# yeyupiaoling/VoiceprintRecognition-PaddlePaddle

Measured on AMD Instinct MI355X. Metric: utterances/sec (3 s, 16 kHz) ECAPA-TDNN fwd+AAM, higher is better.
Workload: dtype bf16; 1 GPU; BASELINE configs[1]: ECAPA-TDNN (C=512, MFA 1536, ASP, embd 192) + Kaldi Fbank 80, 3 s @ 16 kHz (T=298), 2796-class cosine head + AAMLoss, eval-mode forward, batch 256 per GPU, inputs resident in HBM, random-init weights; batch_per_gpu=256, global_batch=256, parallelism=dp1 (no collective), streams_per_gpu=2, hip_graph=True, graph_prereplays=40

## Files before the change

voiceprintrecognition-paddlepaddle_amd/csrc/head_tiled.hip:

```cpp
#include "head_common.h"

#include <math.h>

namespace {

constexpr int HT_CT = 64;
constexpr int HT_RB = 64;
constexpr int HT_RF = 32;
constexpr int HT_DMAX = 256;
constexpr int HT_SW = HT_CT + 2;
typedef __attribute__((ext_vector_type(4))) float v4f;

struct HeadTileArgs {
    const float* emb; const float* W; const long long* labels;
    float* part;
    float* tgt;
    float* cinv;
    const float* rinv;
    int B, D, C, tiles, SE;
    VpMargin mg; float scale; int easy;
    const float* mt;
};

__device__ __forceinline__ float row16_sum(float x) {
    x += __int_as_float(__builtin_amdgcn_update_dpp(0, __float_as_int(x), 0x128, 0xf, 0xf, false));
    x += __int_as_float(__builtin_amdgcn_update_dpp(0, __float_as_int(x), 0x124, 0xf, 0xf, false));
    x += __int_as_float(__builtin_amdgcn_update_dpp(0, __float_as_int(x), 0x122, 0xf, 0xf, false));
    x += __int_as_float(__builtin_amdgcn_update_dpp(0, __float_as_int(x), 0x121, 0xf, 0xf, false));
    return x;
}
__device__ __forceinline__ float row16_max(float x) {
    x = fmaxf(x, __int_as_float(__builtin_amdgcn_update_dpp(0, __float_as_int(x), 0x128, 0xf, 0xf, false)));
    x = fmaxf(x, __int_as_float(__builtin_amdgcn_update_dpp(0, __float_as_int(x), 0x124, 0xf, 0xf, false)));
    x = fmaxf(x, __int_as_float(__builtin_amdgcn_update_dpp(0, __float_as_int(x), 0x122, 0xf, 0xf, false)));
    x = fmaxf(x, __int_as_float(__builtin_amdgcn_update_dpp(0, __float_as_int(x), 0x121, 0xf, 0xf, false)));
    return x;
}


typedef __attribute__((ext_vector_type(4))) unsigned int ht_u32x4;
constexpr unsigned HT_OOB = 0xfffffff0u;

template <int NR>
__device__ __forceinline__ void ht_load_w(const float* W, int D, int C, int c0, int tid, float* Ws) {
    const int cq = (tid & 15) * 4, k0 = tid >> 4;
    if ((C & 3) == 0) {
        const __amdgpu_buffer_rsrc_t srd = __builtin_amdgcn_make_buffer_rsrc(const_cast<float*>(W), 0, (unsigned)((size_t)D * C * 4), 0x00020000);
        const bool cok = c0 + cq < C;
        ht_u32x4 v[NR];
#pragma unroll
        for (int i = 0; i < NR; ++i) {
            const int k = k0 + 16 * i;
            v[i] = __builtin_amdgcn_raw_buffer_load_b128(srd, (cok && k < D) ? (unsigned)(((size_t)k * C + c0 + cq) * 4) : HT_OOB, 0, 0);
        }
#pragma unroll
        for (int i = 0; i < NR; ++i) {
            const int k = k0 + 16 * i;
            if (k < D) {
                float* dst = Ws + k * HT_SW + cq;
                const ht_u32x4 t = v[i];
                dst[0] = __builtin_bit_cast(float, (unsigned)t[0]); dst[1] = __builtin_bit_cast(float, (unsigned)t[1]);
                dst[2] = __builtin_bit_cast(float, (unsigned)t[2]); dst[3] = __builtin_bit_cast(float, (unsigned)t[3]);
            }
        }
    } else {
        for (int k = k0; k < D; k += 16)
#pragma unroll
            for (int e = 0; e < 4; ++e) Ws[k * HT_SW + cq + e] = c0 + cq + e < C ? W[(size_t)k * C + c0 + cq + e] : 0.f;
    }
}

template <int NE, int ROWS = HT_RB>
__device__ __forceinline__ void ht_issue_e(const float* emb, int B, int D, int b0, int tid, ht_u32x4 (&v)[NE]) {
    const __amdgpu_buffer_rsrc_t srd = __builtin_amdgcn_make_buffer_rsrc(const_cast<float*>(emb), 0, (unsigned)((size_t)B * D * 4), 0x00020000);
    const int per_row = D >> 2, total = ROWS * per_row;
#pragma unroll
    for (int i = 0; i < NE; ++i) {
        const int idx = tid + 256 * i;
        const int r = idx / per_row, kq = (idx - r * per_row) * 4;
        v[i] = __builtin_amdgcn_raw_buffer_load_b128(srd, (idx < total && b0 + r < B) ? (unsigned)(((size_t)(b0 + r) * D + kq) * 4) : HT_OOB, 0, 0);
    }
}
template <int NE, int ROWS = HT_RB>
__device__ __forceinline__ void ht_commit_e(int D, int SE, int tid, float* Es, const ht_u32x4 (&v)[NE]) {
    const int per_row = D >> 2, total = ROWS * per_row;
#pragma unroll
    for (int i = 0; i < NE; ++i) {
        const int idx = tid + 256 * i;
        if (idx < total) {
            const int r = idx / per_row, kq = (idx - r * per_row) * 4;
            float* dst = Es + r * SE + kq;
            const ht_u32x4 t = v[i];
            dst[0] = __builtin_bit_cast(float, (unsigned)t[0]); dst[1] = __builtin_bit_cast(float, (unsigned)t[1]);
            dst[2] = __builtin_bit_cast(float, (unsigned)t[2]); dst[3] = __builtin_bit_cast(float, (unsigned)t[3]);
        }
    }
}
template <int NE, int ROWS = HT_RB>
__device__ __forceinline__ void ht_load_e(const float* emb, int B, int D, int SE, int b0, int tid, float* Es) {
    ht_u32x4 v[NE];
    ht_issue_e<NE, ROWS>(emb, B, D, b0, tid, v);
    ht_commit_e<NE, ROWS>(D, SE, tid, Es, v);
}

__global__ __launch_bounds__(256, 2) void head_tile_fwd_kernel(HeadTileArgs a) {
    extern __shared__ __attribute__((aligned(16))) char smem[];
    float* Ws = reinterpret_cast<float*>(smem);
    float* Es = Ws + a.D * HT_SW;
    float* cinv_s = Es + HT_RF * a.SE;
    float* rinv_s = cinv_s + HT_CT;
    float* red = rinv_s + HT_RF;
    int* lab_s = reinterpret_cast<int*>(red + 5 * 4 * HT_RF);
    vp_margin_override(a.mg, a.mt, false);
    const int tid = threadIdx.x, lane = tid & 63, wv = tid >> 6;
    const int li = lane & 15, g = lane >> 4;
    const int tile = blockIdx.x, c0 = tile * HT_CT;
    ht_load_w<HT_DMAX / 16>(a.W, a.D, a.C, c0, tid, Ws);
    __syncthreads();
    {
        const int c = tid & 63, q = tid >> 6;
        float s = 0.f;
        for (int k = q; k < a.D; k += 4) { const float v = Ws[k * HT_SW + c]; s += v * v; }
        red[q * 64 + c] = s;
        __syncthreads();
        if (tid < 64) {
            const float t = red[c] + red[64 + c] + red[128 + c] + red[192 + c];
            const float inv = 1.f / fmaxf(sqrtf(t), 1e-12f);
            cinv_s[c] = inv;
            if (a.cinv && c0 + c < a.C) a.cinv[c0 + c] = inv;
        }
    }
    const int cw = wv * 16;
    constexpr int NE = HT_RF * HT_DMAX / 4 / 256;
    ht_u32x4 ev[NE];
    if ((int)(blockIdx.y * HT_RF) < a.B) ht_issue_e<NE, HT_RF>(a.emb, a.B, a.D, blockIdx.y * HT_RF, tid, ev);
    for (int b0 = blockIdx.y * HT_RF; b0 < a.B; b0 += gridDim.y * HT_RF) {
        __syncthreads();
        if (tid < HT_RF) {
            lab_s[tid] = b0 + tid < a.B ? (int)a.labels[b0 + tid] : -1;
            rinv_s[tid] = b0 + tid < a.B ? a.rinv[b0 + tid] : 0.f;
        }
        ht_commit_e<NE, HT_RF>(a.D, a.SE, tid, Es, ev);
        __syncthreads();
        if (b0 + (int)gridDim.y * HT_RF < a.B) ht_issue_e<NE, HT_RF>(a.emb, a.B, a.D, b0 + gridDim.y * HT_RF, tid, ev);
        constexpr int MI = HT_RF / 16;
        v4f acc[MI];
#pragma unroll
        for (int mi = 0; mi < MI; ++mi) acc[mi] = v4f{0.f, 0.f, 0.f, 0.f};
        const float* wp = Ws + g * HT_SW + cw + li;
        const float* ep = Es + li * a.SE + g;
        const int se16 = 16 * a.SE;
        for (int k = 0; k < a.D; k += 16) {
            float bv[4], av[4][MI];
#pragma unroll
            for (int u = 0; u < 4; ++u) {
                const int kk = k + 4 * u < a.D ? k + 4 * u : 0;
                bv[u] = k + 4 * u < a.D ? wp[kk * HT_SW] : 0.f;
#pragma unroll
                for (int mi = 0; mi < MI; ++mi) av[u][mi] = ep[mi * se16 + kk];
            }
#pragma unroll
            for (int u = 0; u < 4; ++u)
#pragma unroll
                for (int mi = 0; mi < MI; ++mi) acc[mi] = __builtin_amdgcn_mfma_f32_16x16x4f32(av[u][mi], bv[u], acc[mi], 0, 0, 0);
        }
        const int c = c0 + cw + li;
        const bool cvalid = c < a.C;
        const float ci = cinv_s[cw + li];
#pragma unroll
        for (int mi = 0; mi < MI; ++mi) {
#pragma unroll
            for (int r = 0; r < 4; ++r) {
                const int row = mi * 16 + g * 4 + r;
                const int b = b0 + row;
                const int y = lab_s[row];
                const float cs = acc[mi][r] * rinv_s[row] * ci;
                float o = cs;
                if (c == y) o = vp_aam_margin(a.mg, a.easy, cs);
                o *= a.scale;
                if (c == y) a.tgt[b] = o;
                const float ov = cvalid ? o : -INFINITY;
                const float m = row16_max(ov);
                const float s = row16_sum(cvalid ? expf(o - m) : 0.f);
                const float so = row16_sum(cvalid ? o : 0.f);
                const float cv = cvalid ? cs : -INFINITY;
                const float bc = row16_max(cv);
                const float bi = -row16_max(cv == bc ? -(float)c : -INFINITY);
                if (li == 0) {
                    red[(0 * 4 + wv) * HT_RF + row] = m; red[(1 * 4 + wv) * HT_RF + row] = s; red[(2 * 4 + wv) * HT_RF + row] = so;
                    red[(3 * 4 + wv) * HT_RF + row] = bc; red[(4 * 4 + wv) * HT_RF + row] = bi;
                }
            }
        }
        __syncthreads();
        if (tid < HT_RF && b0 + tid < a.B) {
            const int row = tid;
            float M = fmaxf(fmaxf(red[0 * HT_RF + row], red[1 * HT_RF + row]), fmaxf(red[2 * HT_RF + row], red[3 * HT_RF + row]));
            float S = 0.f, O = 0.f;
#pragma unroll
            for (int w = 0; w < 4; ++w) {
                const float mw = red[(0 * 4 + w) * HT_RF + row];
                S += mw == -INFINITY ? 0.f : red[(1 * 4 + w) * HT_RF + row] * expf(mw - M);
                O += red[(2 * 4 + w) * HT_RF + row];
            }
            float BC = -INFINITY, BI = 0.f;
#pragma unroll
            for (int w = 0; w < 4; ++w) {
                const float v = red[(3 * 4 + w) * HT_RF + row];
                if (v > BC) { BC = v; BI = red[(4 * 4 + w) * HT_RF + row]; }
            }
            const size_t o = (size_t)(b0 + row) * a.tiles + tile;
            const size_t st = (size_t)a.B * a.tiles;
            a.part[o] = M;
            a.part[st + o] = S;
            a.part[2 * st + o] = O;
            a.part[3 * st + o] = BC;
            a.part[4 * st + o] = BI;
        }
    }
}

__global__ __launch_bounds__(256) void head_tile_merge_kernel(const float* part, const float* tgt, int B, int C, int tiles, float ls,
                                                              float* lse_out, float* row_loss, int* pred) {
    __shared__ float sm[5][4];
    const int b = blockIdx.x, tid = threadIdx.x, lane = tid & 63, wv = tid >> 6;
    const float* pm = part + (size_t)b * tiles;
    const float* ps = part + (size_t)B * tiles + (size_t)b * tiles;
    const float* po = part + 2 * (size_t)B * tiles + (size_t)b * tiles;
    const float* pc = part + 3 * (size_t)B * tiles + (size_t)b * tiles;
    const float* pi = part + 4 * (size_t)B * tiles + (size_t)b * tiles;
    float mx = -INFINITY, se = 0.f, so = 0.f, bc = -INFINITY, bi = 0.f;
    for (int t = tid; t < tiles; t += 256) {
        const float m = pm[t], s = ps[t];
        so += po[t];
        if (m > mx) { se = se * expf(mx - m) + s; mx = m; }
        else if (m != -INFINITY) se += s * expf(m - mx);
        const float v = pc[t];
        if (v > bc) { bc = v; bi = pi[t]; }
    }
    const float wbc = vp_wave_max(bc);
    const float wbi = -vp_wave_max(bc == wbc ? -bi : -INFINITY);
    if (lane == 0) { sm[3][wv] = wbc; sm[4][wv] = wbi; }
    float lse, O;
    vp_lse_merge(mx, se, so, sm, lse, O);
    if (tid == 0) {
        if (lse_out) lse_out[b] = lse;
        row_loss[b] = (1.f - ls) * (lse - tgt[b]) + ls * (lse - O / (float)C);
        if (pred) {
            float BC = -INFINITY, BI = 0.f;
            for (int w = 0; w < 4; ++w)
                if (sm[3][w] > BC || (sm[3][w] == BC && sm[4][w] < BI)) { BC = sm[3][w]; BI = sm[4][w]; }
            pred[b] = (int)BI;
        }
    }
}

constexpr int HT_SG = HT_CT + 2;

struct HeadBwdArgs {
    const float* emb; const float* W; const long long* labels; const float* lse;
    float* dW; float* dxn_part;
    int B, D, C, tiles, SE;
    VpMargin mg; float scale, ls, gscale; int easy;
    const float* mt;
};

template <int NKB>
__global__ __launch_bounds__(256) void head_tile_bwd_kernel(HeadBwdArgs a) {
    constexpr int D = 16 * NKB;
    constexpr int SE = D + 2;
    constexpr int KPW = NKB / 4;
    extern __shared__ __attribute__((aligned(16))) char smem[];
    float* Ws = reinterpret_cast<float*>(smem);
    float* Es = Ws + D * HT_SW;
    float* Gs = Es + HT_RB * SE;
    float* cinv_s = Gs + HT_RB * HT_SG;
    float* rinv_s = cinv_s + HT_CT;
    float* lse_s = rinv_s + HT_RB;
    float* red = lse_s + HT_RB;
    int* lab_s = reinterpret_cast<int*>(red + 4 * 64);
    vp_margin_override(a.mg, a.mt, false);
    const int tid = threadIdx.x, lane = tid & 63, wv = tid >> 6;
    const int li = lane & 15, g = lane >> 4;
    const int cw = wv * 16;
    const float kk = a.gscale / (float)a.B * a.scale;
    const float qoff = a.ls / (float)a.C;
    const int nrb = (a.B + HT_RB - 1) / HT_RB;
    v4f dxn[2][4][KPW];
#pragma unroll
    for (int rb = 0; rb < 2; ++rb)
#pragma unroll
        for (int mi = 0; mi < 4; ++mi)
#pragma unroll
            for (int kb = 0; kb < KPW; ++kb) dxn[rb][mi][kb] = v4f{0.f, 0.f, 0.f, 0.f};
    for (int tile = blockIdx.x; tile < a.tiles; tile += gridDim.x) {
        const int c0 = tile * HT_CT;
        __syncthreads();
        ht_load_w<NKB>(a.W, D, a.C, c0, tid, Ws);
        __syncthreads();
        {
            const int c = tid & 63, q = tid >> 6;
            float s = 0.f;
            for (int k = q; k < D; k += 4) { const float v = Ws[k * HT_SW + c]; s += v * v; }
            red[q * 64 + c] = s;
            __syncthreads();
            if (tid < 64) cinv_s[c] = 1.f / fmaxf(sqrtf(red[c] + red[64 + c] + red[128 + c] + red[192 + c]), 1e-12f);
        }
        v4f dwn[NKB];
#pragma unroll
        for (int kb = 0; kb < NKB; ++kb) dwn[kb] = v4f{0.f, 0.f, 0.f, 0.f};
#pragma unroll
        for (int rb = 0; rb < 2; ++rb) {
            if (rb < nrb) {
                const int b0 = rb * HT_RB;
                __syncthreads();
                if (tid < HT_RB) {
                    const bool ok = b0 + tid < a.B;
                    lab_s[tid] = ok ? (int)a.labels[b0 + tid] : -1;
                    lse_s[tid] = ok ? a.lse[b0 + tid] : 0.f;
                }
                ht_load_e<HT_RB * D / 4 / 256>(a.emb, a.B, D, SE, b0, tid, Es);
                __syncthreads();
                {
                    const int r = tid & 63, q = tid >> 6;
                    float s = 0.f;
                    for (int k = q; k < D; k += 4) { const float v = Es[r * SE + k]; s += v * v; }
                    red[q * 64 + r] = s;
                    __syncthreads();
                    if (tid < 64) rinv_s[r] = 1.f / fmaxf(sqrtf(red[r] + red[64 + r] + red[128 + r] + red[192 + r]), 1e-12f);
                    __syncthreads();
                }
                v4f acc[4];
#pragma unroll
                for (int mi = 0; mi < 4; ++mi) acc[mi] = v4f{0.f, 0.f, 0.f, 0.f};
                {
                    const float* wp = Ws + g * HT_SW + cw + li;
                    const float* ep = Es + li * SE + g;
                    for (int k = 0; k < D; k += 16) {
                        float bv[4], av[4][4];
#pragma unroll
                        for (int u = 0; u < 4; ++u) {
                            bv[u] = wp[(k + 4 * u) * HT_SW];
#pragma unroll
                            for (int mi = 0; mi < 4; ++mi) av[u][mi] = ep[mi * 16 * SE + k + 4 * u];
                        }
#pragma unroll
                        for (int u = 0; u < 4; ++u)
#pragma unroll
                            for (int mi = 0; mi < 4; ++mi) acc[mi] = __builtin_amdgcn_mfma_f32_16x16x4f32(av[u][mi], bv[u], acc[mi], 0, 0, 0);
                    }
                }
                {
                    const int c = c0 + cw + li;
                    const bool cvalid = c < a.C;
                    const float ci = cinv_s[cw + li];
#pragma unroll
                    for (int mi = 0; mi < 4; ++mi)
#pragma unroll
                        for (int r = 0; r < 4; ++r) {
                            const int row = mi * 16 + g * 4 + r;
                            const int y = lab_s[row];
                            const float cs = acc[mi][r] * rinv_s[row] * ci;
                            float o = cs, dm = 1.f;
                            if (c == y) o = vp_aam_margin(a.mg, a.easy, cs, dm);
                            o *= a.scale;
                            const float q = qoff + (c == y ? 1.f - a.ls : 0.f);
                            const float gv = (cvalid && y >= 0) ? kk * (expf(o - lse_s[row]) - q) * dm * ci : 0.f;
                            Gs[row * HT_SG + cw + li] = gv;
                        }
                }
                __syncthreads();
                {
                    const float* ap = Es + g * SE + li;
                    const float* bp = Gs + g * HT_SG + cw + li;
                    for (int b = 0; b < HT_RB; b += 4) {
                        const float bv = bp[b * HT_SG] * rinv_s[b + g];
                        float av[NKB];
#pragma unroll
                        for (int kb = 0; kb < NKB; ++kb) av[kb] = ap[b * SE + kb * 16];
#pragma unroll
                        for (int kb = 0; kb < NKB; ++kb) dwn[kb] = __builtin_amdgcn_mfma_f32_16x16x4f32(av[kb], bv, dwn[kb], 0, 0, 0);
                    }
                }
                {
                    const float* ap = Gs + li * HT_SG + g;
                    const float* bp = Ws + (wv * KPW * 16 + li) * HT_SW + g;
                    for (int c = 0; c < HT_CT; c += 4) {
                        float av[4], bv[KPW];
#pragma unroll
                        for (int mi = 0; mi < 4; ++mi) av[mi] = ap[mi * 16 * HT_SG + c];
#pragma unroll
                        for (int kb = 0; kb < KPW; ++kb) bv[kb] = bp[kb * 16 * HT_SW + c];
#pragma unroll
                        for (int mi = 0; mi < 4; ++mi)
#pragma unroll
                            for (int kb = 0; kb < KPW; ++kb)
                                dxn[rb][mi][kb] = __builtin_amdgcn_mfma_f32_16x16x4f32(av[mi], bv[kb], dxn[rb][mi][kb], 0, 0, 0);
                    }
                }
            }
        }
        {
            float t = 0.f;
#pragma unroll
            for (int kb = 0; kb < NKB; ++kb)
#pragma unroll
                for (int r = 0; r < 4; ++r) t += Ws[(kb * 16 + g * 4 + r) * HT_SW + cw + li] * dwn[kb][r];
            t += __shfl_xor(t, 16);
            t += __shfl_xor(t, 32);
            const float ci = cinv_s[cw + li];
            t *= ci * ci;
            const int c = c0 + cw + li;
            if (c < a.C) {
#pragma unroll
                for (int kb = 0; kb < NKB; ++kb)
#pragma unroll
                    for (int r = 0; r < 4; ++r) {
                        const int k = kb * 16 + g * 4 + r;
                        a.dW[(size_t)k * a.C + c] = dwn[kb][r] - Ws[k * HT_SW + cw + li] * t;
                    }
            }
        }
    }
    float* out = a.dxn_part + (size_t)blockIdx.x * a.B * D;
#pragma unroll
    for (int rb = 0; rb < 2; ++rb)
#pragma unroll
        for (int mi = 0; mi < 4; ++mi)
#pragma unroll
            for (int kb = 0; kb < KPW; ++kb)
#pragma unroll
                for (int r = 0; r < 4; ++r) {
                    const int b = rb * HT_RB + mi * 16 + g * 4 + r;
                    if (b < a.B) out[(size_t)b * D + (wv * KPW + kb) * 16 + li] = dxn[rb][mi][kb][r];
                }
}

__global__ __launch_bounds__(256) void head_dx_finish_kernel(const float* emb, const float* part, int nparts, int B, int D, float* demb) {
    __shared__ float sm[4];
    const int b = blockIdx.x, tid = threadIdx.x;
    float x = 0.f, gsum = 0.f;
    if (tid < D) {
        x = emb[(size_t)b * D + tid];
        for (int p = 0; p < nparts; ++p) gsum += part[((size_t)p * B + b) * D + tid];
    }
    float n2 = vp_wave_sum(x * x), dt = vp_wave_sum(x * gsum);
    if ((tid & 63) == 0) { sm[tid >> 6] = n2; }
    __syncthreads();
    const float nn = sm[0] + sm[1] + sm[2] + sm[3];
    __syncthreads();
    if ((tid & 63) == 0) { sm[tid >> 6] = dt; }
    __syncthreads();
    const float dot = sm[0] + sm[1] + sm[2] + sm[3];
    const float rinv = 1.f / fmaxf(sqrtf(nn), 1e-12f);
    if (tid < D) demb[(size_t)b * D + tid] = rinv * (gsum - x * rinv * rinv * dot);
}

}

extern "C" {

size_t vp_cosine_aam_tiled_workspace_bytes(int B, int D, int C) {
    (void)D;
    const size_t tiles = (size_t)(C + HT_CT - 1) / HT_CT;
    return vp_align_up(5 * (size_t)B * tiles * 4, 256) + 2 * vp_align_up((size_t)B * 4, 256);
}

int vp_cosine_aam_tiled_fwd(vp_ctx* ctx, const float* emb, const float* W, const int64_t* labels, int B, int D, int C, float margin,
                            float scale, float label_smoothing, int easy_margin, float* loss, float* row_loss, float* lse,
                            float* cinv, int* pred, void* ws, size_t ws_bytes, vp_stream stream) {
    if (!ctx || !emb || !W || !labels || !loss || !row_loss || B <= 0 || C <= 0) VP_FAIL(ctx, VP_EINVAL, "cosine_aam_tiled: bad arguments");
    if (C >= (1 << 24)) VP_FAIL(ctx, VP_EUNSUP, "cosine_aam_tiled: %d classes (class indices travel as exact f32)", C);
    if ((unsigned long long)D * C * 4 >= 0xfffffff0ull || (unsigned long long)B * D * 4 >= 0xfffffff0ull)
        VP_FAIL(ctx, VP_EUNSUP, "cosine_aam_tiled: W (%d x %d) or emb larger than 4 GiB", D, C);
    if (D < 4 || D > HT_DMAX || (D & 3)) VP_FAIL(ctx, VP_EUNSUP, "cosine_aam_tiled: embedding width %d (multiples of 4 up to %d)", D, HT_DMAX);
    if (!ws || ws_bytes < vp_cosine_aam_tiled_workspace_bytes(B, D, C)) VP_FAIL(ctx, VP_EWORKSPACE, "cosine_aam_tiled: workspace too small");
    hipStream_t st = (hipStream_t)stream;
    HeadTileArgs a;
    a.emb = emb; a.W = W; a.labels = (const long long*)labels;
    a.tiles = (C + HT_CT - 1) / HT_CT;
    a.part = (float*)ws;
    a.tgt = (float*)((char*)ws + vp_align_up(5 * (size_t)B * a.tiles * 4, 256));
    a.cinv = cinv;
    float* rinv = (float*)((char*)a.tgt + vp_align_up((size_t)B * 4, 256));
    { const int rc = vp_row_inv_norm(ctx, emb, B, D, D, 1e-12f, rinv, st); if (rc != VP_OK) return rc; }
    a.rinv = rinv;
    a.B = B; a.D = D; a.C = C; a.SE = D + 2;
    a.mg = vp_margin_of(margin);
    a.scale = scale; a.easy = easy_margin; a.mt = ctx->margin_table;
    const int smem = (D * HT_SW + HT_RF * (D + 2) + HT_CT + HT_RF + 5 * 4 * HT_RF + HT_RF) * 4;
    static bool attr_set[64] = {};
    bool& attr_dev = attr_set[ctx->device & 63];
    if (!attr_dev) {
        VP_HIP(ctx, hipFuncSetAttribute(reinterpret_cast<const void*>(head_tile_fwd_kernel), hipFuncAttributeMaxDynamicSharedMemorySize,
                                        (HT_DMAX * HT_SW + HT_RF * (HT_DMAX + 2) + HT_CT + HT_RF + 5 * 4 * HT_RF + HT_RF) * 4));
        attr_dev = true;
    }
    const int rblocks = (B + HT_RF - 1) / HT_RF;
    int ysplit = 1;
    while (ysplit < rblocks && a.tiles * ysplit < 192) ++ysplit;
    hipLaunchKernelGGL(head_tile_fwd_kernel, dim3(a.tiles, ysplit), dim3(256), smem, st, a);
    VP_LAUNCH_CHECK(ctx, "head_tile_fwd");
    hipLaunchKernelGGL(head_tile_merge_kernel, dim3(B), dim3(256), 0, st, a.part, a.tgt, B, C, a.tiles, label_smoothing, lse, row_loss, pred);
    VP_LAUNCH_CHECK(ctx, "head_tile_merge");
    return vp_reduce_rows(ctx, row_loss, B, 1, loss, st);
}

size_t vp_cosine_aam_tiled_bwd_workspace_bytes(int B, int D, int C) {
    const size_t tiles = (size_t)(C + HT_CT - 1) / HT_CT;
    const size_t nwg = tiles < 256 ? tiles : 256;
    return vp_cosine_aam_tiled_workspace_bytes(B, D, C) + vp_align_up((size_t)B * 4, 256) * 2 + vp_align_up(nwg * (size_t)B * D * 4, 256);
}

int vp_cosine_aam_tiled_bwd(vp_ctx* ctx, const float* emb, const float* W, const int64_t* labels, int B, int D, int C, float margin,
                            float scale, float label_smoothing, int easy_margin, float grad_scale, float* demb, float* dW, float* loss,
                            int* pred, void* ws, size_t ws_bytes, vp_stream stream) {
    if (!ctx || !emb || !W || !labels || !demb || !dW || B <= 0 || C <= 0) VP_FAIL(ctx, VP_EINVAL, "cosine_aam_tiled_bwd: bad arguments");
    if (B > 2 * HT_RB || D != 192) return VP_EUNSUP;
    if (!ws || ws_bytes < vp_cosine_aam_tiled_bwd_workspace_bytes(B, D, C)) VP_FAIL(ctx, VP_EWORKSPACE, "cosine_aam_tiled_bwd: workspace too small");
    hipStream_t st = (hipStream_t)stream;
    char* p = (char*)ws;
    const size_t fw = vp_cosine_aam_tiled_workspace_bytes(B, D, C);
    void* fws = p; p += fw;
    float* row_loss = (float*)p; p += vp_align_up((size_t)B * 4, 256);
    float* lse = (float*)p; p += vp_align_up((size_t)B * 4, 256);
    float* part = (float*)p;
    float* loss_dst = loss ? loss : row_loss;
    int rc = vp_cosine_aam_tiled_fwd(ctx, emb, W, labels, B, D, C, margin, scale, label_smoothing, easy_margin, loss_dst, row_loss, lse,
                                     nullptr, pred, fws, fw, stream);
    if (rc) return rc;
    HeadBwdArgs a;
    a.emb = emb; a.W = W; a.labels = (const long long*)labels; a.lse = lse; a.dW = dW; a.dxn_part = part;
    a.B = B; a.D = D; a.C = C; a.tiles = (C + HT_CT - 1) / HT_CT; a.SE = D + 2;
    a.mg = vp_margin_of(margin);
    a.scale = scale; a.ls = label_smoothing; a.gscale = grad_scale; a.easy = easy_margin; a.mt = ctx->margin_table;
    const int nwg = a.tiles < 256 ? a.tiles : 256;
    const int smem = (D * HT_SW + HT_RB * (D + 2) + HT_RB * HT_SG + 64 * 3 + 4 * 64 + 64) * 4;
    static bool attr_set[64] = {};
    bool& attr_dev = attr_set[ctx->device & 63];
    if (!attr_dev) {
        VP_HIP(ctx, hipFuncSetAttribute(reinterpret_cast<const void*>(head_tile_bwd_kernel<12>), hipFuncAttributeMaxDynamicSharedMemorySize,
                                        (192 * HT_SW + HT_RB * 194 + HT_RB * HT_SG + 64 * 3 + 4 * 64 + 64) * 4));
        attr_dev = true;
    }
    hipLaunchKernelGGL(head_tile_bwd_kernel<12>, dim3(nwg), dim3(256), smem, st, a);
    VP_LAUNCH_CHECK(ctx, "head_tile_bwd");
    hipLaunchKernelGGL(head_dx_finish_kernel, dim3(B), dim3(256), 0, st, emb, part, nwg, B, D, demb);
    VP_LAUNCH_CHECK(ctx, "head_dx_finish");
    return VP_OK;
}

}
```

voiceprintrecognition-paddlepaddle_amd/csrc/small_ops.hip:

```cpp
#include "common.h"

#include <stdlib.h>

#include <type_traits>

namespace {

struct MomArgs {
    const float* psum; const float* psumsq; const float* shift; float* stats;
    int B, T, C, nseg, want_std; float eps;
    const float* scale;
};

__global__ __launch_bounds__(256) void moments_kernel(MomArgs a) {
    const int b = blockIdx.y;
    const int c = blockIdx.x * 256 + threadIdx.x;
    if (c >= a.C) return;
    const int t0 = (int)(((long long)b * a.T) / VP_CONV_BM);
    const int t1 = (int)(((long long)(b + 1) * a.T - 1) / VP_CONV_BM);
    float s1 = 0.f, s2 = 0.f;
    for (int tm = t0; tm <= t1; ++tm) {
        const int sg = b - (int)(((long long)tm * VP_CONV_BM) / a.T);
        const size_t idx = ((size_t)tm * a.nseg + sg) * a.C + c;
        s1 += a.psum[idx];
// ... 241 lines not shown
            const int t = (int)(m - b * a.T);
            int ts = t - a.pad + j * a.dil;
            ts = ts < 0 ? -ts : ts;
            ts = ts >= a.T ? 2 * (a.T - 1) - ts : ts;
            const float* src = a.x + ((size_t)b * a.T + ts) * a.F + c;
            *reinterpret_cast<float4*>(v) = *reinterpret_cast<const float4*>(src);
            *reinterpret_cast<float4*>(v + 4) = *reinterpret_cast<const float4*>(src + 4);
        }
        unsigned oh[4], ol[4];
#pragma unroll
        for (int e = 0; e < 4; ++e) {
            const bf16_t h0 = (bf16_t)v[2 * e], h1 = (bf16_t)v[2 * e + 1];
            const bf16_t l0 = (bf16_t)(v[2 * e] - (float)h0), l1 = (bf16_t)(v[2 * e + 1] - (float)h1);
            oh[e] = (unsigned)__builtin_bit_cast(unsigned short, h0) | ((unsigned)__builtin_bit_cast(unsigned short, h1) << 16);
            ol[e] = (unsigned)__builtin_bit_cast(unsigned short, l0) | ((unsigned)__builtin_bit_cast(unsigned short, l1) << 16);
        }
        char* op = a.out + (size_t)m * a.Kp * 4 + (k0 >> 5) * 128 + (k0 & 31) * 2;
        *reinterpret_cast<uint4*>(op) = make_uint4(oh[0], oh[1], oh[2], oh[3]);
        *reinterpret_cast<uint4*>(op + 64) = make_uint4(ol[0], ol[1], ol[2], ol[3]);
    }
}

}

static int se_scale_residual_impl(vp_ctx* ctx, int dtype, const void* x, int ldx, int xoff, const float* s,
                                  const void* res, int ldr, int roff, void* out, int ldo, int ooff, int B, int T, int C,
                                  int relu, void* shadow, int ld_shadow, int shadow_off, hipStream_t st) {
    if (!ctx || !x || !s || !res || !out || B <= 0 || T <= 0 || C <= 0) VP_FAIL(ctx, VP_EINVAL, "se: bad arguments");
    if (shadow && (dtype != VP_F32 || (ld_shadow | shadow_off) & 3 || reinterpret_cast<uintptr_t>(shadow) & 7))
        VP_FAIL(ctx, VP_EINVAL, "se: the bf16 shadow goes with f32 tensors, ld / offset multiples of 4");
    const int V = dtype == VP_HL32 ? 32 : dtype == VP_BF16 ? 8 : 4;
    if (C % V || ldx % V || xoff % V || ldr % V || roff % V || ldo % V || ooff % V)
        VP_FAIL(ctx, VP_EINVAL, "se: C/ld/off must be multiples of %d", V);
    if ((reinterpret_cast<uintptr_t>(x) | reinterpret_cast<uintptr_t>(res) | reinterpret_cast<uintptr_t>(out) | reinterpret_cast<uintptr_t>(s)) & 15)
        VP_FAIL(ctx, VP_EINVAL, "se: tensors must be 16-byte aligned");
    if (dtype == VP_HL32) {
        const long long tot = (long long)B * T * (C / 8);
        long long nb = (tot + 255) / 256;
        if (nb > 256 * 16) nb = 256 * 16;
        SeHlArgs a{(const char*)x, s, (const char*)res, (char*)out, ldx, xoff, ldr, roff, ldo, ooff, T, C, relu, tot};
        hipLaunchKernelGGL(se_scale_residual_hl_kernel, dim3((unsigned)nb), dim3(256), 0, st, a);
        VP_LAUNCH_CHECK(ctx, "se_scale_residual_hl");
        return VP_OK;
    }
    const long long total = (long long)B * T * (C / V);
    long long blocks = (total + 255) / 256;
    if (blocks > 256 * 16) blocks = 256 * 16;
    if (dtype == VP_BF16) {
        SeArgs<bf16_t> a{(const bf16_t*)x, s, (const bf16_t*)res, (bf16_t*)out, ldx, xoff, ldr, roff, ldo, ooff, T, C, relu, total, nullptr, 0, 0};
        hipLaunchKernelGGL(se_scale_residual_kernel<bf16_t>, dim3((unsigned)blocks), dim3(256), 0, st, a);
    } else if (dtype == VP_F32) {
        SeArgs<float> a{(const float*)x, s, (const float*)res, (float*)out, ldx, xoff, ldr, roff, ldo, ooff, T, C, relu, total,
                        (bf16_t*)shadow, ld_shadow, shadow_off};
        hipLaunchKernelGGL(se_scale_residual_kernel<float>, dim3((unsigned)blocks), dim3(256), 0, st, a);
    } else {
        VP_FAIL(ctx, VP_EINVAL, "se: bad dtype");
    }
    VP_LAUNCH_CHECK(ctx, "se_scale_residual");
    return VP_OK;
}

int vp_se_scale_residual_ex(vp_ctx* ctx, int dtype, const void* x, int ldx, int xoff, const float* s,
                            const void* res, int ldr, int roff, void* out, int ldo, int ooff, int B, int T, int C,
                            int relu, hipStream_t st) {
    return se_scale_residual_impl(ctx, dtype, x, ldx, xoff, s, res, ldr, roff, out, ldo, ooff, B, T, C, relu, nullptr, 0, 0, st);
}

int vp_im2col_hl32(vp_ctx* ctx, const float* x, int B, int T, int F, int KW, int dil, int pad, void* out, int Kp, hipStream_t st) {
    if (!ctx || !x || !out || B <= 0 || T <= 0 || F % 8 || Kp % 32 || Kp < KW * F || pad >= T || dil * (KW - 1) - pad >= T ||
        (reinterpret_cast<uintptr_t>(x) | reinterpret_cast<uintptr_t>(out)) & 15)
        VP_FAIL(ctx, VP_EINVAL, "im2col_hl32: bad arguments");
    const long long total = (long long)B * T * (Kp / 8);
    long long nb = (total + 255) / 256;
    if (nb > 256 * 32) nb = 256 * 32;
    Im2colArgs a{x, (char*)out, T, F, KW, dil, pad, Kp, total};
    hipLaunchKernelGGL(im2col_hl_kernel, dim3((unsigned)nb), dim3(256), 0, st, a);
    VP_LAUNCH_CHECK(ctx, "im2col_hl32");
    return VP_OK;
}

namespace {
template <typename T>
struct CopyArgs { const T* x; T* y; int ldx, xoff, ldy, yoff, C4; long long total; };
template <typename T>
__global__ __launch_bounds__(256) void copy_cols_kernel(CopyArgs<T> a) {
    for (long long i = (long long)blockIdx.x * 256 + threadIdx.x; i < a.total; i += (long long)gridDim.x * 256) {
        const long long r = i / a.C4;
        const int c = (int)(i - r * a.C4) * 4;
        float v[4];
        vp_load4(a.x + r * a.ldx + a.xoff + c, v);
        vp_store4(a.y + r * a.ldy + a.yoff + c, v);
    }
}
template <typename T>
struct AffArgs { const T* t; const T* x; const T* y; T* o; int ldt, ldx, xoff, ldy, yoff, ldo, ooff, C4; long long total; };
template <typename T>
__global__ __launch_bounds__(256) void aff_combine_kernel(AffArgs<T> a) {
    for (long long i = (long long)blockIdx.x * 256 + threadIdx.x; i < a.total; i += (long long)gridDim.x * 256) {
        const long long r = i / a.C4;
        const int c = (int)(i - r * a.C4) * 4;
        float t[4], x[4], y[4], o[4];
        vp_load4(a.t + r * a.ldt + c, t);
        vp_load4(a.x + r * a.ldx + a.xoff + c, x);
        vp_load4(a.y + r * a.ldy + a.yoff + c, y);
#pragma unroll
        for (int e = 0; e < 4; ++e) o[e] = x[e] * (1.f + t[e]) + y[e] * (1.f - t[e]);
        vp_store4(a.o + r * a.ldo + a.ooff + c, o);
    }
}
unsigned grid_for(long long total) {
    long long b = (total + 255) / 256;
    return (unsigned)(b > 256 * 64 ? 256 * 64 : (b < 1 ? 1 : b));
}
}

int vp_copy_cols(vp_ctx* ctx, int dtype, const void* x, int ldx, int xoff, void* y, int ldy, int yoff, long long rows, int C,
                 hipStream_t st) {
    if ((C | ldx | xoff | ldy | yoff) & 3) VP_FAIL(ctx, VP_EINVAL, "copy_cols: widths / offsets must be multiples of 4");
    const long long total = rows * (C / 4);
    if (dtype == VP_BF16) {
        CopyArgs<bf16_t> a{(const bf16_t*)x, (bf16_t*)y, ldx, xoff, ldy, yoff, C / 4, total};
        hipLaunchKernelGGL(copy_cols_kernel<bf16_t>, dim3(grid_for(total)), dim3(256), 0, st, a);
    } else {
        CopyArgs<float> a{(const float*)x, (float*)y, ldx, xoff, ldy, yoff, C / 4, total};
        hipLaunchKernelGGL(copy_cols_kernel<float>, dim3(grid_for(total)), dim3(256), 0, st, a);
    }
    VP_LAUNCH_CHECK(ctx, "copy_cols");
    return VP_OK;
}

int vp_aff_combine(vp_ctx* ctx, int dtype, const void* t, int ldt, const void* x, int ldx, int xoff, const void* y, int ldy,
                   int yoff, void* o, int ldo, int ooff, long long rows, int C, hipStream_t st) {
    if ((C | ldt | ldx | xoff | ldy | yoff | ldo | ooff) & 3) VP_FAIL(ctx, VP_EINVAL, "aff_combine: widths / offsets must be multiples of 4");
    const long long total = rows * (C / 4);
    if (dtype == VP_BF16) {
        AffArgs<bf16_t> a{(const bf16_t*)t, (const bf16_t*)x, (const bf16_t*)y, (bf16_t*)o, ldt, ldx, xoff, ldy, yoff, ldo, ooff, C / 4, total};
        hipLaunchKernelGGL(aff_combine_kernel<bf16_t>, dim3(grid_for(total)), dim3(256), 0, st, a);
    } else {
        AffArgs<float> a{(const float*)t, (const float*)x, (const float*)y, (float*)o, ldt, ldx, xoff, ldy, yoff, ldo, ooff, C / 4, total};
        hipLaunchKernelGGL(aff_combine_kernel<float>, dim3(grid_for(total)), dim3(256), 0, st, a);
    }
    VP_LAUNCH_CHECK(ctx, "aff_combine");
    return VP_OK;
}

namespace {
struct SeGateArgs {
    const float* psum; const float* shift; const float* w1; const float* b1; const float* w2; const float* b2; float* out;
    int B, T, C, H, nseg;
};

constexpr int SE_UPW = 1;

__device__ __forceinline__ void se_matvec(const float* in, int ldi, int K, const float* W, int N, const float* bias, int sigmoid,
                                          float* out, int ldo, float* part) {
    const int tid = threadIdx.x, nt = blockDim.x;
    const int nv = N >> 2;
    const int ns = nt / nv;
    const int v = tid % nv, sl = tid / nv;
    if (sl < ns) {
        const int k0 = (int)((long long)K * sl / ns), k1 = (int)((long long)K * (sl + 1) / ns);
        float4 acc[SE_UPW];
#pragma unroll
        for (int u = 0; u < SE_UPW; ++u) acc[u] = make_float4(0.f, 0.f, 0.f, 0.f);
        const float* wp = W + 4 * v;
#pragma unroll 8
        for (int k = k0; k < k1; ++k) {
            const float4 w = *reinterpret_cast<const float4*>(wp + (size_t)k * N);
#pragma unroll
            for (int u = 0; u < SE_UPW; ++u) {
                const float x = in[u * ldi + k];
                acc[u].x += x * w.x; acc[u].y += x * w.y; acc[u].z += x * w.z; acc[u].w += x * w.w;
            }
        }
#pragma unroll
        for (int u = 0; u < SE_UPW; ++u) *reinterpret_cast<float4*>(part + (u * ns + sl) * N + 4 * v) = acc[u];
    }
    __syncthreads();
    for (int i = tid; i < SE_UPW * N; i += nt) {
        const int u = i / N, n = i - u * N;
        float acc = bias ? bias[n] : 0.f;
        for (int q = 0; q < ns; ++q) acc += part[(u * ns + q) * N + n];
        out[u * ldo + n] = sigmoid ? 1.f / (1.f + __expf(-acc)) : fmaxf(acc, 0.f);
    }
}

__global__ __launch_bounds__(1024) void se_gate_kernel(SeGateArgs a) {
    extern __shared__ float sm[];
    float* mean = sm;
    float* h = mean + SE_UPW * a.C;
    float* sg = h + SE_UPW * a.H;
    float* part = sg + SE_UPW * a.C;
    const int b0 = blockIdx.x * SE_UPW;
    {
        const int groups = max(1, (int)blockDim.x / (SE_UPW * a.C));
        const int i = threadIdx.x % (SE_UPW * a.C), gq = threadIdx.x / (SE_UPW * a.C);
        const int u = i / a.C, c = i - u * a.C;
        const int b = min(b0 + u, a.B - 1);
        const int t0 = (int)(((long long)b * a.T) / VP_CONV_BM);
        const int t1 = (int)(((long long)(b + 1) * a.T - 1) / VP_CONV_BM);
        for (int i2 = i; i2 < SE_UPW * a.C; i2 += blockDim.x) {
            const int u2 = i2 / a.C, c2 = i2 - u2 * a.C;
            float s1 = 0.f;
            if (gq < groups) {
#pragma unroll 4
                for (int tm = t0 + gq; tm <= t1; tm += groups) {
                    const int seg = b - (int)(((long long)tm * VP_CONV_BM) / a.T);
                    s1 += a.psum[((size_t)tm * a.nseg + seg) * a.C + c2];
                }
            }
            if (groups == 1) { if (gq == 0) mean[i2] = (a.shift ? a.shift[c2] : 0.f) + s1 / (float)a.T; }
            else if (gq < groups) part[gq * (SE_UPW * a.C) + i2] = s1;
            (void)u2;
        }
        if (groups > 1) {
            __syncthreads();
            if (gq == 0) {
                float s1 = 0.f;
                for (int q = 0; q < groups; ++q) s1 += part[q * (SE_UPW * a.C) + i];
                mean[i] = (a.shift ? a.shift[c] : 0.f) + s1 / (float)a.T;
            }
        }
        (void)u;
    }
    __syncthreads();
    se_matvec(mean, a.C, a.C, a.w1, a.H, a.b1, 0, h, a.H, part);
    __syncthreads();
    se_matvec(h, a.H, a.H, a.w2, a.C, a.b2, 1, sg, a.C, part);
    __syncthreads();
    for (int i = threadIdx.x; i < SE_UPW * a.C; i += blockDim.x) {
        const int u = i / a.C;
        if (b0 + u < a.B) a.out[(size_t)(b0 + u) * a.C + (i - u * a.C)] = sg[i];
    }
}
}

int vp_se_gate(vp_ctx* ctx, const float* psum, const float* shift, int B, int T, int C, int H, const float* w1, const float* b1,
               const float* w2, const float* b2, float* out, hipStream_t st) {
    if (!psum || !w1 || !w2 || !out || B <= 0 || T <= 0 || C <= 0 || H <= 0) VP_FAIL(ctx, VP_EINVAL, "se_gate: bad arguments");
    if ((C | H) & 3 || C > 1024 || H > 1024) VP_FAIL(ctx, VP_EUNSUP, "se_gate: C %d / H %d (multiples of 4, <= 1024)", C, H);
    constexpr int SE_THREADS = 1024;
    const size_t smem = (size_t)SE_UPW * (2 * C + H + 4 * SE_THREADS) * sizeof(float);
    if (smem > 64 * 1024) VP_FAIL(ctx, VP_EUNSUP, "se_gate: %d channels do not fit the LDS budget", C);
    SeGateArgs a{psum, shift, w1, b1, w2, b2, out, B, T, C, H, vp_conv1d_nseg(T)};
    hipLaunchKernelGGL(se_gate_kernel, dim3((B + SE_UPW - 1) / SE_UPW), dim3(SE_THREADS), smem, st, a);
    VP_LAUNCH_CHECK(ctx, "se_gate");
    return VP_OK;
}

int vp_dense_f32_ex(vp_ctx* ctx, const float* a, int lda, const float* w, int w_is_kn, const float* bias,
                    const float* rowscale, const float* colscale, int M, int N, int K, int act, float* out,
                    int ldo, hipStream_t st) {
    if (!a || !w || !out || M <= 0 || N <= 0 || K <= 0) VP_FAIL(ctx, VP_EINVAL, "dense: bad arguments");
    DenseArgs p;
    p.a = a; p.w = w; p.bias = bias; p.rowscale = rowscale; p.colscale = colscale; p.out = out;
    p.lda = lda; p.ldo = ldo; p.M = M; p.N = N; p.K = K; p.w_is_kn = w_is_kn; p.act = act;
    const int nw = K >= 1024 ? 16 : 4;
    p.kper = ((K + nw - 1) / nw + 15) / 16 * 16;
    p.vec_ok = (lda % 4 == 0) && ((reinterpret_cast<uintptr_t>(a) & 15) == 0);
    p.wvec_ok = (K % 4 == 0) && ((reinterpret_cast<uintptr_t>(w) & 15) == 0);
    dim3 grid((N + 15) / 16, (M + 15) / 16);
    if (grid.y > 65535) VP_FAIL(ctx, VP_EINVAL, "dense: M too large");
    hipLaunchKernelGGL(dense_f32_kernel, grid, dim3(64 * nw), 0, st, p);
    VP_LAUNCH_CHECK(ctx, "dense_f32");
    return VP_OK;
}

int vp_row_inv_norm(vp_ctx* ctx, const float* x, int rows, int D, int ld, float eps, float* inv, hipStream_t st) {
    hipLaunchKernelGGL(row_inv_norm_kernel, dim3((rows + 3) / 4), dim3(256), 0, st, x, rows, D, ld, eps, inv);
    VP_LAUNCH_CHECK(ctx, "row_inv_norm");
    return VP_OK;
}

extern "C" {

int vp_moments_finalize_affine(vp_ctx* ctx, const float* psum, const float* psumsq, const float* scale, const float* shift,
                               int B, int T, int C, float eps, int want_std, float* stats, vp_stream stream) {
    if (!ctx || !psum || !stats || !scale || !shift || (want_std && !psumsq) || B <= 0 || T <= 0 || C <= 0)
        VP_FAIL(ctx, VP_EINVAL, "moments: bad arguments");
    if (B > 65535) VP_FAIL(ctx, VP_EINVAL, "moments: batch too large");
    MomArgs a;
    a.psum = psum; a.psumsq = psumsq; a.shift = shift; a.scale = scale; a.stats = stats; a.B = B; a.T = T; a.C = C;
    a.nseg = vp_conv1d_nseg(T); a.want_std = want_std; a.eps = eps;
    hipLaunchKernelGGL(moments_kernel, dim3((C + 255) / 256, B), dim3(256), 0, (hipStream_t)stream, a);
    VP_LAUNCH_CHECK(ctx, "moments");
    return VP_OK;
}

int vp_moments_finalize(vp_ctx* ctx, const float* psum, const float* psumsq, const float* shift,
                        int B, int T, int C, float eps, int want_std, float* stats, vp_stream stream) {
    if (!ctx || !psum || !stats || (want_std && !psumsq) || B <= 0 || T <= 0 || C <= 0)
        VP_FAIL(ctx, VP_EINVAL, "moments: bad arguments");
    if (B > 65535) VP_FAIL(ctx, VP_EINVAL, "moments: batch too large");
    MomArgs a;
    a.psum = psum; a.psumsq = psumsq; a.shift = shift; a.scale = nullptr; a.stats = stats; a.B = B; a.T = T; a.C = C;
    a.nseg = vp_conv1d_nseg(T); a.want_std = want_std; a.eps = eps;
    hipLaunchKernelGGL(moments_kernel, dim3((C + 255) / 256, B), dim3(256), 0, (hipStream_t)stream, a);
    VP_LAUNCH_CHECK(ctx, "moments");
    return VP_OK;
}

int vp_dense_f32(vp_ctx* ctx, const float* a, int lda, const float* w, int w_is_kn, const float* bias,
                 int M, int N, int K, int act, float* out, int ldo, vp_stream stream) {
    if (!ctx) return VP_EINVAL;
    return vp_dense_f32_ex(ctx, a, lda, w, w_is_kn, bias, nullptr, nullptr, M, N, K, act, out, ldo, (hipStream_t)stream);
}

int vp_se_scale_residual_shadow(vp_ctx* ctx, const float* x, int ldx, int xoff, const float* s, const float* res, int ldr, int roff,
                                float* out, int ldo, int ooff, void* shadow, int ld_shadow, int shadow_off, int B, int T, int C,
                                vp_stream stream) {
    return se_scale_residual_impl(ctx, VP_F32, x, ldx, xoff, s, res, ldr, roff, out, ldo, ooff, B, T, C, 0, shadow, ld_shadow, shadow_off,
                                  (hipStream_t)stream);
}

int vp_se_scale_residual_z16(vp_ctx* ctx, const void* z, int ldz, const float* bn_scale, const float* bn_shift, const float* s, const void* res,
                             int ldr, int roff, void* out, int ldo, int ooff, int B, int T, int C, vp_stream stream) {
    if (!ctx || !z || !bn_scale || !bn_shift || !s || !res || !out || B <= 0 || T <= 0 || C <= 0) VP_FAIL(ctx, VP_EINVAL, "se_z16: bad arguments");
    if (C % 8 || ldz % 8 || ldr % 8 || roff % 8 || ldo % 8 || ooff % 8 ||
        ((reinterpret_cast<uintptr_t>(z) | reinterpret_cast<uintptr_t>(res) | reinterpret_cast<uintptr_t>(out) | reinterpret_cast<uintptr_t>(s) |
          reinterpret_cast<uintptr_t>(bn_scale) | reinterpret_cast<uintptr_t>(bn_shift)) & 15))
        VP_FAIL(ctx, VP_EINVAL, "se_z16: C / ld / offsets must be multiples of 8, tensors 16-byte aligned");
    const long long total = (long long)B * T * (C / 8);
    long long blocks = (total + 255) / 256;
    if (blocks > 256 * 16) blocks = 256 * 16;
    SeZArgs a{(const bf16_t*)z, bn_scale, bn_shift, s, (const bf16_t*)res, (bf16_t*)out, ldz, ldr, roff, ldo, ooff, T, C, total};
    hipLaunchKernelGGL(se_scale_residual_z16_kernel, dim3((unsigned)blocks), dim3(256), 0, (hipStream_t)stream, a);
    VP_LAUNCH_CHECK(ctx, "se_scale_residual_z16");
    return VP_OK;
}

int vp_se_scale_residual(vp_ctx* ctx, int dtype, const void* x, int ldx, int xoff, const float* s,
                         const void* res, int ldr, int roff, void* out, int ldo, int ooff,
                         int B, int T, int C, vp_stream stream) {
    return vp_se_scale_residual_ex(ctx, dtype, x, ldx, xoff, s, res, ldr, roff, out, ldo, ooff, B, T, C, 0, (hipStream_t)stream);
}

}

namespace {
__global__ __launch_bounds__(256) void cast_bf16_kernel(const float* x, bf16_t* y, long long n) {
    for (long long i = ((long long)blockIdx.x * 256 + threadIdx.x) * 4; i < n; i += (long long)gridDim.x * 1024) {
        if (i + 3 < n) {
            float4 v = *reinterpret_cast<const float4*>(x + i);
            bf16x4 o;
            o[0] = (bf16_t)v.x; o[1] = (bf16_t)v.y; o[2] = (bf16_t)v.z; o[3] = (bf16_t)v.w;
            *reinterpret_cast<bf16x4*>(y + i) = o;
        } else {
            for (long long j = i; j < n; ++j) y[j] = (bf16_t)x[j];
        }
    }
}
}

extern "C" int vp_cast_f32_bf16(vp_ctx* ctx, const float* x, void* y, long long n, vp_stream stream) {
    if (!ctx || !x || !y || n <= 0) VP_FAIL(ctx, VP_EINVAL, "cast: bad arguments");
    if ((reinterpret_cast<uintptr_t>(x) & 15) || (reinterpret_cast<uintptr_t>(y) & 7)) VP_FAIL(ctx, VP_EINVAL, "cast: misaligned");
    long long blocks = (n / 4 + 255) / 256;
    if (blocks > 4096) blocks = 4096;
    if (blocks < 1) blocks = 1;
    hipLaunchKernelGGL(cast_bf16_kernel, dim3((unsigned)blocks), dim3(256), 0, (hipStream_t)stream, x, (bf16_t*)y, n);
    VP_LAUNCH_CHECK(ctx, "cast_bf16");
    return VP_OK;
}
```

Baseline: 196,700 utterances/s.

## Fuse row norms and loss mean into head kernels; prefetch SE weights

```diff
diff --git a/voiceprintrecognition-paddlepaddle_amd/csrc/head_tiled.hip b/voiceprintrecognition-paddlepaddle_amd/csrc/head_tiled.hip
--- a/voiceprintrecognition-paddlepaddle_amd/csrc/head_tiled.hip
+++ b/voiceprintrecognition-paddlepaddle_amd/csrc/head_tiled.hip
@@ -16,7 +16,7 @@
     float* part;
     float* tgt;
     float* cinv;
-    const float* rinv;
+    int* counter;
     int B, D, C, tiles, SE;
     VpMargin mg; float scale; int easy;
     const float* mt;
@@ -115,6 +115,7 @@
     const int tid = threadIdx.x, lane = tid & 63, wv = tid >> 6;
     const int li = lane & 15, g = lane >> 4;
     const int tile = blockIdx.x, c0 = tile * HT_CT;
+    if (tid == 0 && blockIdx.x == 0 && blockIdx.y == 0) *a.counter = 0;
     ht_load_w<HT_DMAX / 16>(a.W, a.D, a.C, c0, tid, Ws);
     __syncthreads();
     {
@@ -136,13 +137,27 @@
     if ((int)(blockIdx.y * HT_RF) < a.B) ht_issue_e<NE, HT_RF>(a.emb, a.B, a.D, blockIdx.y * HT_RF, tid, ev);
     for (int b0 = blockIdx.y * HT_RF; b0 < a.B; b0 += gridDim.y * HT_RF) {
         __syncthreads();
-        if (tid < HT_RF) {
-            lab_s[tid] = b0 + tid < a.B ? (int)a.labels[b0 + tid] : -1;
-            rinv_s[tid] = b0 + tid < a.B ? a.rinv[b0 + tid] : 0.f;
-        }
+        if (tid < HT_RF) lab_s[tid] = b0 + tid < a.B ? (int)a.labels[b0 + tid] : -1;
         ht_commit_e<NE, HT_RF>(a.D, a.SE, tid, Es, ev);
         __syncthreads();
         if (b0 + (int)gridDim.y * HT_RF < a.B) ht_issue_e<NE, HT_RF>(a.emb, a.B, a.D, b0 + gridDim.y * HT_RF, tid, ev);
+        {
+            constexpr int NR = HT_RF / 4;
+            float s[NR];
+#pragma unroll
+            for (int j = 0; j < NR; ++j) {
+                s[j] = 0.f;
+                for (int d = lane; d < a.D; d += 64) { const float v = Es[(wv + 4 * j) * a.SE + d]; s[j] += v * v; }
+            }
+#pragma unroll
+            for (int o = 32; o > 0; o >>= 1)
+#pragma unroll
+                for (int j = 0; j < NR; ++j) s[j] += __shfl_xor(s[j], o);
+            float mine = s[0];
+#pragma unroll
+            for (int j = 1; j < NR; ++j) mine = lane == j ? s[j] : mine;
+            if (lane < NR) rinv_s[wv + 4 * lane] = b0 + wv + 4 * lane < a.B ? 1.f / fmaxf(sqrtf(mine), 1e-12f) : 0.f;
+        }
         constexpr int MI = HT_RF / 16;
         v4f acc[MI];
 #pragma unroll
@@ -164,6 +179,7 @@
 #pragma unroll
                 for (int mi = 0; mi < MI; ++mi) acc[mi] = __builtin_amdgcn_mfma_f32_16x16x4f32(av[u][mi], bv[u], acc[mi], 0, 0, 0);
         }
+        __syncthreads();
         const int c = c0 + cw + li;
         const bool cvalid = c < a.C;
         const float ci = cinv_s[cw + li];
@@ -221,8 +237,10 @@
 }
 
 __global__ __launch_bounds__(256) void head_tile_merge_kernel(const float* part, const float* tgt, int B, int C, int tiles, float ls,
-                                                              float* lse_out, float* row_loss, int* pred) {
+                                                              float* lse_out, float* row_loss, int* pred, int* counter, float* loss) {
     __shared__ float sm[5][4];
+    __shared__ float sm_mean[4];
+    __shared__ int last_s;
     const int b = blockIdx.x, tid = threadIdx.x, lane = tid & 63, wv = tid >> 6;
     const float* pm = part + (size_t)b * tiles;
     const float* ps = part + (size_t)B * tiles + (size_t)b * tiles;
@@ -252,6 +270,19 @@
                 if (sm[3][w] > BC || (sm[3][w] == BC && sm[4][w] < BI)) { BC = sm[3][w]; BI = sm[4][w]; }
             pred[b] = (int)BI;
         }
+        last_s = __hip_atomic_fetch_add(counter, 1, __ATOMIC_ACQ_REL, __HIP_MEMORY_SCOPE_AGENT) == B - 1;
+    }
+    __syncthreads();
+    if (!last_s) return;
+    float s = 0.f;
+    for (int i = tid; i < B; i += 256) s += __hip_atomic_load(row_loss + i, __ATOMIC_RELAXED, __HIP_MEMORY_SCOPE_AGENT);
+    s = vp_wave_sum(s);
+    if (lane == 0) sm_mean[wv] = s;
+    __syncthreads();
+    if (tid == 0) {
+        const float t = sm_mean[0] + sm_mean[1] + sm_mean[2] + sm_mean[3];
+        loss[0] = t / (float)B;
+        __hip_atomic_store(counter, 0, __ATOMIC_RELAXED, __HIP_MEMORY_SCOPE_AGENT);
     }
 }
 
@@ -482,9 +513,7 @@
     a.part = (float*)ws;
     a.tgt = (float*)((char*)ws + vp_align_up(5 * (size_t)B * a.tiles * 4, 256));
     a.cinv = cinv;
-    float* rinv = (float*)((char*)a.tgt + vp_align_up((size_t)B * 4, 256));
-    { const int rc = vp_row_inv_norm(ctx, emb, B, D, D, 1e-12f, rinv, st); if (rc != VP_OK) return rc; }
-    a.rinv = rinv;
+    a.counter = (int*)((char*)a.tgt + vp_align_up((size_t)B * 4, 256));
     a.B = B; a.D = D; a.C = C; a.SE = D + 2;
     a.mg = vp_margin_of(margin);
     a.scale = scale; a.easy = easy_margin; a.mt = ctx->margin_table;
@@ -501,9 +530,10 @@
     while (ysplit < rblocks && a.tiles * ysplit < 192) ++ysplit;
     hipLaunchKernelGGL(head_tile_fwd_kernel, dim3(a.tiles, ysplit), dim3(256), smem, st, a);
     VP_LAUNCH_CHECK(ctx, "head_tile_fwd");
-    hipLaunchKernelGGL(head_tile_merge_kernel, dim3(B), dim3(256), 0, st, a.part, a.tgt, B, C, a.tiles, label_smoothing, lse, row_loss, pred);
+    hipLaunchKernelGGL(head_tile_merge_kernel, dim3(B), dim3(256), 0, st, a.part, a.tgt, B, C, a.tiles, label_smoothing, lse, row_loss, pred,
+                       a.counter, loss);
     VP_LAUNCH_CHECK(ctx, "head_tile_merge");
-    return vp_reduce_rows(ctx, row_loss, B, 1, loss, st);
+    return VP_OK;
 }
 
 size_t vp_cosine_aam_tiled_bwd_workspace_bytes(int B, int D, int C) {
diff --git a/voiceprintrecognition-paddlepaddle_amd/csrc/small_ops.hip b/voiceprintrecognition-paddlepaddle_amd/csrc/small_ops.hip
--- a/voiceprintrecognition-paddlepaddle_amd/csrc/small_ops.hip
+++ b/voiceprintrecognition-paddlepaddle_amd/csrc/small_ops.hip
@@ -417,20 +417,44 @@
 
 constexpr int SE_UPW = 1;
 
-__device__ __forceinline__ void se_matvec(const float* in, int ldi, int K, const float* W, int N, const float* bias, int sigmoid,
-                                          float* out, int ldo, float* part) {
+constexpr int SE_PRE = 16;
+
+template <int J0, int J1>
+__device__ __forceinline__ void se_w_issue(const float* W, int K, int N, float4 (&w)[SE_PRE]) {
+    const int tid = threadIdx.x, nt = blockDim.x;
+    const int nv = N >> 2, ns = nt / nv;
+    const int v = tid % nv, sl = tid / nv;
+    const int k0 = K * sl / ns;
+    const float* wp = W + 4 * v;
+#pragma unroll
+    for (int j = J0; j < J1; ++j) w[j] = *reinterpret_cast<const float4*>(wp + (size_t)min(k0 + j, K - 1) * N);
+}
+
+__device__ __forceinline__ void se_matvec_part(const float* in, int ldi, int K, const float* W, int N, const float4 (&wr)[SE_PRE], float* part) {
     const int tid = threadIdx.x, nt = blockDim.x;
     const int nv = N >> 2;
     const int ns = nt / nv;
     const int v = tid % nv, sl = tid / nv;
     if (sl < ns) {
-        const int k0 = (int)((long long)K * sl / ns), k1 = (int)((long long)K * (sl + 1) / ns);
+        const int k0 = K * sl / ns, k1 = K * (sl + 1) / ns;
         float4 acc[SE_UPW];
 #pragma unroll
         for (int u = 0; u < SE_UPW; ++u) acc[u] = make_float4(0.f, 0.f, 0.f, 0.f);
         const float* wp = W + 4 * v;
+#pragma unroll
+        for (int j = 0; j < SE_PRE; ++j) {
+            const int k = k0 + j;
+            if (k < k1) {
+                const float4 w = wr[j];
+#pragma unroll
+                for (int u = 0; u < SE_UPW; ++u) {
+                    const float x = in[u * ldi + k];
+                    acc[u].x += x * w.x; acc[u].y += x * w.y; acc[u].z += x * w.z; acc[u].w += x * w.w;
+                }
+            }
+        }
 #pragma unroll 8
-        for (int k = k0; k < k1; ++k) {
+        for (int k = k0 + SE_PRE; k < k1; ++k) {
             const float4 w = *reinterpret_cast<const float4*>(wp + (size_t)k * N);
 #pragma unroll
             for (int u = 0; u < SE_UPW; ++u) {
@@ -441,6 +465,11 @@
 #pragma unroll
         for (int u = 0; u < SE_UPW; ++u) *reinterpret_cast<float4*>(part + (u * ns + sl) * N + 4 * v) = acc[u];
     }
+}
+
+__device__ __forceinline__ void se_matvec_finish(int N, const float* bias, int sigmoid, float* out, int ldo, const float* part) {
+    const int tid = threadIdx.x, nt = blockDim.x;
+    const int ns = nt / (N >> 2);
     __syncthreads();
     for (int i = tid; i < SE_UPW * N; i += nt) {
         const int u = i / N, n = i - u * N;
@@ -457,6 +486,8 @@
     float* sg = h + SE_UPW * a.H;
     float* part = sg + SE_UPW * a.C;
     const int b0 = blockIdx.x * SE_UPW;
+    float4 w1r[SE_PRE], w2r[SE_PRE];
+    se_w_issue<0, SE_PRE>(a.w1, a.C, a.H, w1r);
     {
         const int groups = max(1, (int)blockDim.x / (SE_UPW * a.C));
         const int i = threadIdx.x % (SE_UPW * a.C), gq = threadIdx.x / (SE_UPW * a.C);
@@ -489,9 +520,12 @@
         (void)u;
     }
     __syncthreads();
-    se_matvec(mean, a.C, a.C, a.w1, a.H, a.b1, 0, h, a.H, part);
+    se_matvec_part(mean, a.C, a.C, a.w1, a.H, w1r, part);
+    se_w_issue<0, SE_PRE>(a.w2, a.H, a.C, w2r);
+    se_matvec_finish(a.H, a.b1, 0, h, a.H, part);
     __syncthreads();
-    se_matvec(h, a.H, a.H, a.w2, a.C, a.b2, 1, sg, a.C, part);
+    se_matvec_part(h, a.H, a.H, a.w2, a.C, w2r, part);
+    se_matvec_finish(a.C, a.b2, 1, sg, a.C, part);
     __syncthreads();
     for (int i = threadIdx.x; i < SE_UPW * a.C; i += blockDim.x) {
         const int u = i / a.C;
```

Measured after the change: 195,000 utterances/s. About the same (-0.9%).
